# pangenome/seqrush

Hardware: AMD Instinct MI355X
Metric: aligned pairs/sec all-vs-all 64x5kb (higher is better)
Workload: dtype i16; 1 GPU; C2: 64 x 5 kb synthetic (5% SNP, seed 2001), all-vs-all incl. self = 4096 ordered pairs, -k 0 -S 0,5,8,2,24,1 --orientation-scores 0,1,1,1, biWFA (Ultralow); pairs_total=4096, pairs_per_gpu=4096, parallelism=pair-shard x1

## Files before the change

include/seqrush_amd.h:

```cpp
#ifndef SEQRUSH_AMD_H
#define SEQRUSH_AMD_H
#include <stddef.h>
#include <stdint.h>

#ifdef __cplusplus
extern "C" {
#endif

#define SR_ABI_VERSION 2

typedef enum {
    SR_OK = 0,
    SR_ERR_INVALID = -1,
    SR_ERR_NO_DEVICE = -2,
    SR_ERR_HIP = -3,
    SR_ERR_ALPHABET = -4,
    SR_ERR_EMPTY_SEQ = -5,
    SR_ERR_UNSUPPORTED = -6,
    SR_ERR_DEVICE_FAULT = -7,
    SR_ERR_IO = -8,
    SR_ERR_NOMEM = -9
} sr_status;

typedef struct {
// ... 116 lines not shown
    uint64_t random_entries;
    uint64_t random_processed;
    uint64_t random_aligned;
    uint64_t checks;
    uint64_t windows;
    uint64_t post_tree;
    uint64_t final_components;
    int32_t stabilized;
    int32_t tree_defaulted;
    uint32_t tree_k_nearest, tree_k_farthest;
    double tree_rand_frac;
    uint32_t tree_kmer;
    uint32_t reserved;
} sr_iter_stats;
int sr_ctx_load_iterative(sr_ctx *c, const sr_seqset *seqs, const sr_params *p, int keep_alignments);
int sr_ctx_run_iterative(sr_ctx *c);
int sr_ctx_iterative_stats(sr_ctx *c, sr_iter_stats *out, uint64_t *check_counts, uint64_t cap);
int sr_ctx_iterative_alignments(sr_ctx *c, sr_alignments **out);
int sr_uf_count_components_host(const uint64_t *nodes, uint64_t n, uint64_t total_len, uint64_t *count);
int sr_iterative_stop_host(const uint64_t *counts, uint64_t nchecks, uint64_t post_tree, uint64_t *stop_check);
int sr_iterative_pair_lists(uint32_t n, const uint8_t *sel, const sr_params *p, uint32_t **tree_i, uint32_t **tree_j,
                            uint64_t *tree_count, uint32_t **rand_i, uint32_t **rand_j, uint64_t *rand_count);
int sr_base_cone_reach(int e1, int e2, int two, int levels_left);
int sr_mirror_map(const uint32_t *query_idx, const uint32_t *target_idx, uint64_t count, const uint32_t *batch_first,
                  uint32_t nbatch, uint32_t workgroups, uint32_t *mirror_out, uint64_t *partners_out);
int sr_ctx_orientation_scores(sr_ctx *c, int32_t *fwd, int32_t *rev);
int sr_mirror_bt_pick(const int *off, int transposed);
int sr_mirror_bt_rank_transposed(int tag);
int sr_mirror_bt_tie_host(const int *off);
int sr_mirror_bp_pick_host(const int *val, const int *dist, const int *comp, const int *diag, int n, int value_bias,
                           int *pick_out, int *pick_t_out);
int sr_replay_record_ints(void);
void sr_replay_transpose_host(const int *rec, int *out);
int sr_replay_match_host(const int *recs, int nrec, const int *segs, int nseg, int level, int *match_out);

typedef struct {
    uint64_t min_size;
    int32_t keep_alignments;
    uint32_t join_below;
} sr_inv_params;
typedef struct {
    uint64_t scanned;
    uint64_t sites;
    uint64_t candidates;
    uint64_t accepted;
    uint64_t rejected_score;
// ... 217 lines not shown
```

seqrush_amd/_lib.py:

```python
import ctypes as C
import os

_HERE = os.path.dirname(os.path.abspath(__file__))
LIB_PATH = os.environ.get("SEQRUSH_AMD_LIB") or os.path.join(_HERE, "libseqrush_amd.so")

EXPORTS = [
    "sr_default_params", "sr_parse_scores", "sr_parse_orientation_scores",
    "sr_parse_sparsification", "sr_align_all", "sr_alignments_free", "sr_alignment_cigar",
    "sr_align_and_unite", "sr_uf_find", "sr_uf_same", "sr_write_paf", "sr_ctx_create",
    "sr_ctx_destroy", "sr_ctx_set_stream", "sr_ctx_load", "sr_ctx_reset_uf", "sr_ctx_align",
    "sr_ctx_unite", "sr_ctx_sync", "sr_ctx_alignments", "sr_ctx_download_uf", "sr_ctx_uf_size",
    "sr_ctx_num_pairs", "sr_ctx_dp_cells", "sr_ctx_labels_device", "sr_ctx_merge_labels",
    "sr_ctx_download_labels", "sr_ctx_kernel_ms", "sr_ctx_counters", "sr_build_gfa", "sr_free",
    "sr_last_error", "sr_abi_version", "sr_device_count", "sr_pair_list", "sr_ctx_align_kernel",
    "sr_ctx_load_paf", "sr_unite_paf", "sr_ctx_build_gfa", "sr_ctx_load_pairs", "sr_ctx_pairs",
    "sr_ctx_num_batches", "sr_ctx_workspace_report", "sr_ctx_run", "sr_ctx_align_all", "sr_ctx_pair_results",
    "sr_ctx_labels_device_u32", "sr_ctx_merge_labels_u32", "sr_ctx_counters_ext",
    "sr_build_gfa_opts", "sr_ctx_build_gfa_opts", "sr_ctx_merge_labels_host",
    "sr_uf_init_host", "sr_uf_unite_host", "sr_uf_merge_labels_host", "sr_uf_canonical_labels_host",
    "sr_build_gfa_from_nodes", "sr_ctx_counters_all", "sr_knobs_doc",
    "sr_sort_params_default", "sr_ctx_build_gfa_sorted", "sr_sort_gfa", "sr_sgd_layout", "sr_sgd_tables", "sr_sort_stats",
    "sr_ctx_load_iterative", "sr_ctx_run_iterative", "sr_ctx_iterative_stats", "sr_ctx_iterative_alignments",
    "sr_uf_count_components_host", "sr_iterative_stop_host", "sr_iterative_pair_lists", "sr_base_cone_reach",
    "sr_ctx_enable_inversions", "sr_ctx_inversion_stats", "sr_ctx_inversion_jobs", "sr_ctx_inversion_alignments",
    "sr_append_paf_tagged", "sr_inversion_sites_host", "sr_inversion_candidate", "sr_inversion_accept",
    "sr_inversion_scan_device",
    "sr_ctx_inversion_join_stats", "sr_inversion_sites_host_join", "sr_inversion_accept_site", "sr_inversion_scan_device_join",
    "sr_compact_gfa", "sr_compact_stats",
    "sr_sketch_device", "sr_knn_select_device",
    "sr_graph_stats_gfa", "sr_graph_stats_free", "sr_graph_stats_report", "sr_stats_sq_sums_host",
    "sr_mirror_map", "sr_mirror_bt_pick", "sr_mirror_bt_rank_transposed", "sr_mirror_bt_tie_host", "sr_mirror_bp_pick_host",
    "sr_ctx_orientation_scores",
    "sr_layout_params_default", "sr_layout_gfa", "sr_layout_tsv", "sr_layout_svg", "sr_layout_quality", "sr_layout_stats",
    "sr_layout_resolve", "sr_layout_select_host",
    "sr_path_bins_gfa", "sr_path_bins_free", "sr_path_bins_tsv", "sr_viz_params_default", "sr_path_bins_rgb", "sr_path_bins_png",
    "sr_growth_params_default", "sr_growth_gfa", "sr_growth_free", "sr_growth_groups", "sr_growth_expected", "sr_growth_fit",
    "sr_growth_report",
    "sr_variant_params_default", "sr_variants_gfa", "sr_variants_free", "sr_variants_vcf",
    "sr_ctx_tail_deferred", "sr_ctx_tail_timeline", "sr_tail_shape",
    "sr_replay_record_ints", "sr_replay_transpose_host", "sr_replay_match_host",
    "sr_ctx_prio_timeline", "sr_tile_prio_role_host", "sr_tile_prio_epoch_shift",
]


class SeqSetC(C.Structure):
    _fields_ = [("n", C.c_uint32), ("bases", C.c_char_p), ("offsets", C.POINTER(C.c_uint64)),
                ("names", C.POINTER(C.c_char_p))]


class ParamsC(C.Structure):
    _fields_ = [
        ("match_score", C.c_int32), ("mismatch_penalty", C.c_int32),
        ("gap_open1", C.c_int32), ("gap_ext1", C.c_int32),
        ("gap_open2", C.c_int32), ("gap_ext2", C.c_int32),
        ("ori_match", C.c_int32), ("ori_mismatch", C.c_int32),
        ("ori_gap_open", C.c_int32), ("ori_gap_ext", C.c_int32),
        ("min_match_len", C.c_uint64), ("max_divergence", C.c_double),
        ("exclude_self", C.c_int32), ("memory_mode", C.c_int32),
        ("sparsify_kind", C.c_int32), ("sparsify_factor", C.c_double),
        ("sparsify_seed", C.c_uint64), ("canonical_labels", C.c_int32), ("device", C.c_int32),
        ("shard_rank", C.c_uint32), ("shard_count", C.c_uint32),
        ("tree_k_nearest", C.c_uint32), ("tree_k_farthest", C.c_uint32), ("tree_rand_frac", C.c_double),
        ("tree_kmer", C.c_uint32),
    ]
# ... 186 lines not shown
    L.sr_build_gfa_opts.argtypes = [PS, C.POINTER(u64), i32, C.POINTER(vp), C.POINTER(u64), C.POINTER(u64)]
    L.sr_ctx_build_gfa_opts.argtypes = [vp, PS, i32, C.POINTER(vp), C.POINTER(u64), C.POINTER(u64)]
    L.sr_uf_init_host.argtypes = [C.POINTER(u64), u64, u64]
    L.sr_uf_unite_host.argtypes = [C.POINTER(u64), u64, u64, u64]
    L.sr_uf_merge_labels_host.argtypes = [C.POINTER(u64), u64, C.POINTER(u64), C.c_uint32]
    L.sr_uf_canonical_labels_host.argtypes = [C.POINTER(u64), u64, C.POINTER(u64)]
    L.sr_build_gfa_from_nodes.argtypes = [PS, C.POINTER(u64), i32, C.POINTER(vp), C.POINTER(u64), C.POINTER(u64)]
    SP, PD = C.POINTER(SortParamsC), C.POINTER(C.c_double)
    L.sr_sort_params_default.argtypes = [SP]; L.sr_sort_params_default.restype = None
    L.sr_ctx_build_gfa_sorted.argtypes = [vp, PS, i32, SP, C.POINTER(vp), C.POINTER(u64), C.POINTER(u64)]
    L.sr_sort_gfa.argtypes = [C.c_char_p, SP, C.POINTER(vp), C.POINTER(u64), C.POINTER(u64)]
    L.sr_sgd_layout.argtypes = [C.c_char_p, SP, PD, u64]
    L.sr_sgd_tables.argtypes = [C.c_char_p, SP, SP, C.POINTER(u64), PD, PD, PD, PD]
    L.sr_sort_stats.argtypes = [PD, C.c_uint32]
    L.sr_pair_list.argtypes = [C.c_uint32, PP, C.POINTER(C.POINTER(C.c_uint32)),
                               C.POINTER(C.POINTER(C.c_uint32)), C.POINTER(u64)]
    L.sr_ctx_load_iterative.argtypes = [vp, PS, PP, i32]
    L.sr_ctx_run_iterative.argtypes = [vp]
    L.sr_ctx_iterative_stats.argtypes = [vp, C.POINTER(IterStatsC), C.POINTER(u64), u64]
    L.sr_ctx_iterative_alignments.argtypes = [vp, C.POINTER(C.POINTER(AlignmentsC))]
    L.sr_uf_count_components_host.argtypes = [C.POINTER(u64), u64, u64, C.POINTER(u64)]
    L.sr_iterative_stop_host.argtypes = [C.POINTER(u64), u64, u64, C.POINTER(u64)]
    L.sr_base_cone_reach.argtypes = [C.c_int, C.c_int, C.c_int, C.c_int]
    PU32 = C.POINTER(C.POINTER(C.c_uint32))
    L.sr_iterative_pair_lists.argtypes = [C.c_uint32, C.POINTER(C.c_uint8), PP, PU32, PU32, C.POINTER(u64), PU32, PU32,
                                          C.POINTER(u64)]
    L.sr_ctx_enable_inversions.argtypes = [vp, C.POINTER(InvParamsC)]
    L.sr_ctx_inversion_stats.argtypes = [vp, C.POINTER(InvStatsC)]
    L.sr_ctx_inversion_jobs.argtypes = [vp, C.POINTER(C.POINTER(InvJobC)), C.POINTER(u64)]
    L.sr_ctx_inversion_alignments.argtypes = [vp, C.POINTER(C.POINTER(AlignmentsC))]
    L.sr_append_paf_tagged.argtypes = [C.POINTER(AlignmentsC), PS, C.c_char_p, C.c_char_p]
    L.sr_inversion_sites_host.argtypes = [C.POINTER(C.c_uint32), u64, u64, C.POINTER(C.POINTER(InvSiteC)), C.POINTER(u64)]
    L.sr_inversion_candidate.argtypes = [u64, u64, u64]
    L.sr_inversion_accept.argtypes = [C.c_int32, C.c_int32]
    L.sr_inversion_scan_device.argtypes = [i32, C.POINTER(C.c_uint32), C.POINTER(u64), u64, u64,
                                           C.POINTER(C.POINTER(InvSiteC)), C.POINTER(C.POINTER(u64)), C.POINTER(u64)]
    PI32 = C.POINTER(C.c_int32)
    L.sr_ctx_inversion_join_stats.argtypes = [vp, C.POINTER(u64)]
    L.sr_inversion_sites_host_join.argtypes = [C.POINTER(C.c_uint32), u64, u64, C.c_uint32, PP, C.POINTER(C.POINTER(InvSiteC)),
                                               C.POINTER(PI32), C.POINTER(u64)]
    L.sr_inversion_accept_site.argtypes = [C.c_int32, C.c_int32]
    L.sr_inversion_scan_device_join.argtypes = [i32, C.POINTER(C.c_uint32), C.POINTER(u64), u64, u64, C.c_uint32, PP, PI32, PI32,
                                                C.POINTER(C.POINTER(InvSiteC)), C.POINTER(C.POINTER(u64)), C.POINTER(PI32),
                                                C.POINTER(u64), C.POINTER(u64)]
    PU32P = C.POINTER(C.POINTER(C.c_uint32))
    L.sr_sketch_device.argtypes = [i32, PS, C.c_uint32, C.POINTER(C.POINTER(u64)), PU32P, PU32P, PU32P]
# ... 61 lines not shown
```

seqrush_amd/csrc/sr_align_blk.inc:

```
#include "sr_blk_rows.inc"
#include "sr_blk_tile.inc"
#include "sr_blk_pass.inc"
#include "sr_blk_phase2.inc"
#include "sr_blk_orient.inc"

#define K_SHIFT0 29
#define K_WIDTH0 64
struct KSeqs { int poff_f, poff_r, toff_f, toff_r, plen_all, tlen_all; };
__device__ __forceinline__ void kjob_set(int jid, int base, int pb, int pe, int tb, int te, int rev, int begin, int chk,
                                         int seg, const KSeqs &q) {
    bjob_set(jid, base, pb, pe, tb, te, 0, begin, chk, seg, rev ? q.poff_r : q.poff_f);
    BJob &b = b_sh.job[jid];
    b.shift = (pe - pb) + K_SHIFT0;
    b.pad0 = rev ? q.toff_r : q.toff_f;
    b.pad2 = 1;
    if (rev) { b.p0 = q.plen_all - pe; b.t0 = q.tlen_all - te; }
}
__device__ __forceinline__ int kjob_width(int plen, int tlen) { return (plen + tlen + K_WIDTH0) & ~3; }

#define SR_BLK_MIN_WAVES 4
template <typename OT, int NT, bool TWO, int B, int E1, int E2, bool PROF = false, int X = 0, int OE1 = 0, typename RT = OT>
__global__ void __launch_bounds__(NT, SR_BLK_MIN_WAVES) sr_align_blk_kernel(SrAlignArgs a) {
    const int tid = threadIdx.x;
    if (a.tail_mode == SR_TAIL_RUN && *a.tail_count == 0u) return;
// ... 259 lines not shown
                if (RFL(k_sh.rp_ntot) == 0) break;
                any_bp = true;
                if (tid == 0) k_sh.dg_nbp += (unsigned long long)k_sh.rp_ntot;
                if (nact == 0) {
                    if (tid == 0) k_sh.dg_steps += 2ull * (unsigned long long)k_sh.rp_ntot * B * (unsigned long long)k_sh.rp_maxp;
                    continue;
                }
                const unsigned long long tb0 = KTICK();
                const int njobs = 2 * nact;
                for (int s0i = 0; RFL(b_sh.nrunning) > 0; s0i += B) {
                    const int s0 = kopaque_s(s0i);
                    const unsigned long long q0 = KTICK();
                    blk_pass<OT, TWO, NT, B, E1, E2, PROF, X, OE1, RT, true>(RR, s0, pen, njobs, row_ld, row_st, s0 == 0);
                    const unsigned long long q1 = KTICK();
                    __syncthreads();
                    const unsigned long long q2 = KTICK();
                    tq_pass += q1 - q0; tq_bar += q2 - q1;
                    if (tid == 0) k_sh.dg_steps += (unsigned long long)njobs * B;
                    const int avail = s0 + B - 1;
                    const int tid_o = tid;
                    if (tid < 64) {
                        const int tid = (int)kopaque_v((unsigned)tid_o);
                        KPRIO_HI();
                        if (tid < njobs) {
#pragma unroll
                            for (int j = 0; j < B; j++) gmak[tid * BFS_MAK_SLOTS + (s0 + j) % depth] = k_sh.jak[j][tid];
                        }
                        const unsigned long long qc1 = KTICK();
                        int ph = 0, ph0 = 0;
                        if (tid < nact) {
                            BSeg &sg = b_sh.seg[tid];
                            ph = sg.phase; ph0 = ph;
                            const long long smax = 2LL * ((long long)pen.o1 * 2 + (long long)pen.e1 * (sg.max_ad + 1)) + 1024;
                            if (ph == 1) {
                                int score_f = sg.score_f, score_r = sg.score_r, last_fwd = sg.last_fwd, f_ak = sg.f_ak, r_ak = sg.r_ak;
                                const int max_ad = sg.max_ad;
                                for (int j = 0; j < B && ph == 1; j++) {
                                    const int s = s0 + j;
                                    const int akf = k_sh.jak[j][2 * tid], akr = k_sh.jak[j][2 * tid + 1];
                                    if (s == 0) {
                                        f_ak = akf; r_ak = akr;
                                        if (f_ak + r_ak >= max_ad) ph = 2;
                                    } else {
                                        score_f = s; f_ak = akf; last_fwd = 1;
                                        if (f_ak + r_ak >= max_ad) ph = 2;
                                        else {
                                            score_r = s; r_ak = akr; last_fwd = 0;
                                            if ((long long)score_f + score_r > smax) ph = 4;
                                            else if (f_ak + r_ak >= max_ad) ph = 2;
                                        }
                                    }
                                }
                                sg.score_f = score_f; sg.score_r = score_r; sg.last_fwd = last_fwd; sg.f_ak = f_ak; sg.r_ak = r_ak;
                                sg.phase = ph;
                            }
                        }
                        const unsigned long long qc2 = KTICK();
                        if (PROF && tid == 0) { k_sh.t_c1 += qc1 - q2; k_sh.t_c2 += qc2 - qc1; }
                        const unsigned long long m2 = __ballot(ph == 2);
                        const unsigned long long mnew = __ballot(ph == 2 && ph0 == 1);
                        if (tid == 0) k_sh.newmask = (unsigned)mnew;
                        if (tid == 0) { k_sh.p2mask_lo = (unsigned)m2; k_sh.p2mask_hi = (unsigned)(m2 >> 32); }
                        if (m2 == 0ull) {
                            const unsigned long long run = __ballot(ph == 1);
                            if (tid < nact && ph != 1) { b_sh.job[2 * tid].active = 0; b_sh.job[2 * tid + 1].active = 0; }
                            if (tid == 0) b_sh.nrunning = __popcll(run);
                            if (run != 0ull) blk_setup<TWO, NT, B, E1, E2, KTIGHT>(s0 + B, pen, njobs);
                        }
                        KPRIO_LO();
                    }
                    __syncthreads();
                    const unsigned long long q3 = KTICK();
                    tq_ctl += q3 - q2;
                    bool p2_or_rec = (RFL(k_sh.p2mask_lo) | RFL(k_sh.p2mask_hi)) != 0u;
                    if (a.lazy_id) {
                        if (RFL(k_sh.newmask) != 0u) p2_or_rec = true;
                        for (unsigned nm = RFL(k_sh.newmask); nm != 0u; nm &= nm - 1u) {
                            const int sa = __ffs((int)nm) - 1;
                            blk_recompute<OT, TWO, NT, B, E1, E2, X, OE1>(RR, pen, sa, RFL(b_sh.seg[sa].score_f), s0, row_ld, row_st);
                        }
                    }
                    tq_rec += KTICK() - q3;
                    if ((RFL(k_sh.p2mask_lo) | RFL(k_sh.p2mask_hi)) != 0u) {
                        blk_phase2<OT, TWO, NT, B, E1, E2, RT, PROF>(RR, clist, gmak, pen, s0, nact, gap_opening);
                        if (tid < 64) {
                            KPRIO_HI();
                            const int ph = (tid < nact) ? b_sh.seg[tid].phase : 0;
                            const unsigned long long run = __ballot(ph == 1 || ph == 2);
                            if (tid < nact && ph != 1 && ph != 2) { b_sh.job[2 * tid].active = 0; b_sh.job[2 * tid + 1].active = 0; }
                            if (tid == 0) b_sh.nrunning = __popcll(run);
                            if (run != 0ull) blk_setup<TWO, NT, B, E1, E2, KTIGHT>(s0 + B, pen, njobs);
                            KPRIO_LO();
                        }
                    }
                    const unsigned long long q4 = KTICK();
                    if (p2_or_rec) __syncthreads();
                    tq_ph2 += q4 - q3; tq_tail += KTICK() - q4;
                    if (tid == 0) k_sh.dg_npass += 1ull;
                }
                if (tid < nact) {
                    BSeg &sg = b_sh.seg[tid];
                    GP<int> e = cur + (size_t)sg.list_pos * SR_BFS_SEGREC;
                    const int sp = sg.pe - sg.pb, st = sg.te - sg.tb;
                    const int bh = sg.bp_off_f, bv = sg.bp_off_f - sg.bp_k_f;
                    if (sg.phase != 3 || sg.bp_score == INT_MAX) atomicOr(&b_sh.err, SR_DEV_ERR_SCORE_BOUND);
                    else if (bv < 0 || bv > sp || bh < 0 || bh > st) atomicOr(&b_sh.err, SR_DEV_ERR_BREAKPOINT);
                    else {
                        e[SL_BV] = bv; e[SL_BH] = bh; e[SL_BCOMP] = sg.bp_comp; e[SL_BSF] = sg.bp_score_f; e[SL_BSR] = sg.bp_score_r;
                        const int ri = k_sh.rp_nrec + tid;
                        if (k_sh.rp_record != 0 && ri < SR_BPREC_MAX) {
                            GP<int> r = (GP<int>)a.brec + (size_t)blockIdx.x * (SR_BPREC_MAX * SR_BPREC_INTS) + ri * SR_BPREC_INTS;
                            const unsigned long long cs = k_sh.cells_l[2 * tid] + k_sh.cells_l[2 * tid + 1] - (unsigned long long)(long long)k_sh.sg_sur[tid];
                            r[SR_BR_LEVEL] = k_sh.rp_level;
                            r[SR_BR_PB] = sg.pb; r[SR_BR_PE] = sg.pe; r[SR_BR_TB] = sg.tb; r[SR_BR_TE] = sg.te; r[SR_BR_CB] = sg.cb; r[SR_BR_CE] = sg.ce;
// ... 76 lines not shown
                        kjob_set(nb, 0, e[SL_PB], e[SL_PE], e[SL_TB], e[SL_TE], 0, e[SL_CB], ce, nb, ks);
                        b_sh.job[nb].shift = wj / 2;
                        b_sh.job[nb].pad1 = lj;
                        b_sh.job[nb].hbase = (unsigned)used; b_sh.job[nb].hw = (unsigned)wj;
                        b_sh.base_entry[nb] = p; b_sh.base_score[nb] = -1;
                        used += need; lmax = max(lmax, lj);
                        nb++;
                    }
                    b_sh.nbase = nb; b_sh.next_pos = p; b_sh.njobs = nb; b_sh.nrunning = nb;
                    b_sh.geom.hist_levels = lmax;
                }
                __syncthreads();
                int nb = RFL(b_sh.nbase);
                pos = RFL(b_sh.next_pos);
                if (nb > 0) {
                    if (tid == 0) k_sh.dg_nbase += (unsigned long long)nb;
                    const int hlevels = RFL(b_sh.geom.hist_levels);
                    for (int s0i = 0; RFL(b_sh.nrunning) > 0; s0i += B) {
                        const int s0 = kopaque_s(s0i);
                        if (s0 + B > hlevels) { if (tid == 0) b_sh.err |= SR_DEV_ERR_BASE_OVERFLOW; break; }
                        blk_pass<OT, TWO, NT, B, E1, E2, PROF, X, OE1, OT, false, true>(RH, s0, pen, nb, row_ld, row_st, s0 == 0);
                        __syncthreads();
                        if (tid == 0) k_sh.dg_steps += (unsigned long long)b_sh.nrunning * B;
                        if (tid < 64) {
                            KPRIO_HI();
                            bool running = false;
                            if (tid < nb && b_sh.job[tid].active) {
                                int hit = -1;
#pragma unroll
                                for (int l = B - 1; l >= 0; l--) if (k_sh.jreach[l][tid]) hit = l;
                                if (hit >= 0) {
                                    b_sh.base_score[tid] = s0 + hit; b_sh.job[tid].active = 0;
                                    atomicAdd(&b_sh.cells, (unsigned long long)(-blk_surplus(pen, tid, s0 + hit, s0 + B - 1)));
                                } else if (s0 + 2 * B > b_sh.job[tid].pad1) {
                                    GP<int> e = cur + (size_t)b_sh.base_entry[tid] * SR_BFS_SEGREC;
                                    b_sh.job[tid].active = 0;
                                    if (e[SL_REM] < 0 || b_sh.job[tid].pad1 >= a.hist_levels) atomicOr(&b_sh.err, SR_DEV_ERR_BASE_OVERFLOW);
                                    else { e[SL_REM] = -1; atomicMin(&k_sh.redo_from, tid); atomicAdd(&k_sh.dg_redo, 1ull); }
                                } else running = true;
                            }
                            const unsigned long long rm = __ballot(running);
                            if (tid == 0) b_sh.nrunning = __popcll(rm);
                            if (rm != 0ull) blk_setup<TWO, NT, B, E1, E2, false, true>(s0 + B, pen, nb);
                            KPRIO_LO();
                        }
                        __syncthreads();
                    }
                    __syncthreads();
                    const int redo = RFL(k_sh.redo_from);
                    if (redo < nb) {
                        if (tid == 0) k_sh.dg_nbase -= (unsigned long long)(nb - redo);
                        nb = redo; pos = RFL(b_sh.base_entry[redo]);
                    }
                    const unsigned long long tbt0 = KTICK();
                    if (tid < nb && RFL(b_sh.err) == 0) {
                        KPRIO_HI();
                        int n = 0;
                        const int e = bfs_backtrace<OT, TWO>(bhist + b_sh.job[tid].hbase, b_sh.job[tid].hw, tid, b_sh.base_score[tid],
                                                             btbuf + (size_t)tid * SR_BFS_BTCAP, &n);
                        b_sh.bt_n[tid] = n;
                        if (e & SR_MIRROR_BT_TIE) k_sh.mir_tie = 1;
                        if (e & ~SR_MIRROR_BT_TIE) atomicOr(&b_sh.err, e & ~SR_MIRROR_BT_TIE);
                        KPRIO_LO();
                    }
                    __syncthreads();
                    tb_bt += KTICK() - tbt0;
// ... 196 lines not shown
```

seqrush_amd/csrc/sr_blk_pass.inc:

```
#include "sr_base_cone.h"
#include "sr_prio_rule.h"
template <bool TWO, int E1, int E2>
__device__ __forceinline__ int kreach(const SrPen &p, int s, int begin) {
    int r;
    if (begin == SR_C_M) {
        r = (s >= p.o1 + E1) ? (s - p.o1) / E1 : 0;
        if (TWO && s >= p.o2 + E2) r = max(r, (s - p.o2) / E2);
    } else {
        r = s / E1;
        if (TWO) r = max(r, s / E2);
    }
    return r;
}

template <bool TWO, int B, int E1, int E2, bool TIGHT>
__device__ __forceinline__ void kwindow(const SrPen &pen, const BJob &b, int s0, int &glo, int &ghi) {
    const int Rw = kreach<TWO, E1, E2>(pen, s0 + B - 1, b.begin);
    const int mg = TIGHT ? 1 : pen.scope + 1;
    const int wlo = max(-b.plen - 1, -Rw - mg), whi = min(b.tlen + 1, Rw + mg);
    glo = (wlo + b.shift) >> 2; ghi = (whi + b.shift) >> 2;
}

#define KTICK() (PROF ? __builtin_amdgcn_s_memrealtime() : 0ull)
__device__ __forceinline__ void kprio_role() {
    switch (RFL(k_sh.prio_role)) {
    case 1: __builtin_amdgcn_s_setprio(1); break;
    case 2: __builtin_amdgcn_s_setprio(2); break;
    case 3: __builtin_amdgcn_s_setprio(3); break;
    default: __builtin_amdgcn_s_setprio(0); break;
    }
}
__device__ __forceinline__ void kprio_epoch() {
    const int wg = RFL(k_sh.prio_wg);
    if (wg > 1) {
        const unsigned epoch = (unsigned)(__builtin_amdgcn_s_memrealtime() >> SR_PRIO_EPOCH_SHIFT);
        if (threadIdx.x == 0) k_sh.prio_role = sr_tile_prio_role((unsigned)k_sh.prio_rank, epoch, (unsigned)wg);
    }
}
#define KPRIO_HI() __builtin_amdgcn_s_setprio(3)
#define KPRIO_LO() kprio_role()
#ifndef SR_BASE_CONE
#define SR_BASE_CONE 1
#endif
template <bool TWO, int NT, int B, int E1, int E2, bool TIGHT = false, bool BASE = false>
__device__ __forceinline__ void blk_setup(int s0, const SrPen &pen, int njobs) {
    const int tid = threadIdx.x;
    constexpr bool CONE = BASE && SR_BASE_CONE;
    int nt = 0, glo = 0, ghi = -1, cells = 0, ccells = 0;
    const bool act = tid < njobs && b_sh.job[tid].active;
    const int pglo = (tid < BJ_MAX) ? k_sh.jglo[tid] : 0, pghi = (tid < BJ_MAX) ? k_sh.jghi[tid] : -1;
    if (act) {
        const BJob &b = b_sh.job[tid];
        int Rw = 0, clo0 = 0, chi0 = 0;
#pragma unroll
        for (int j = 0; j < B; j++) {
            Rw = kreach<TWO, E1, E2>(pen, s0 + j, b.begin);
            int klo = max(-b.plen, -Rw), khi = min(b.tlen, Rw);
            cells += (khi >= klo) ? khi - klo + 1 : 0;
            if (CONE) {
                const int rb = sr_cone_reach(E1, E2, TWO, b.pad1 - 1 - (s0 + j));
                klo = max(klo, b.kend - rb); khi = min(khi, b.kend + rb);
                if (j == 0) { clo0 = b.kend - rb; chi0 = b.kend + rb; }
            }
            k_sh.jklo[j][tid] = klo; k_sh.jkhi[j][tid] = khi;
            ccells += (khi >= klo) ? khi - klo + 1 : 0;
        }
        (void)Rw;
        kwindow<TWO, B, E1, E2, TIGHT>(pen, b, s0, glo, ghi);
        if (CONE) {
            const int mg = TIGHT ? 1 : pen.scope + 1;
            const int wlo = max(max(-b.plen - 1, -Rw - mg), clo0 - 1), whi = min(min(b.tlen + 1, Rw + mg), chi0 + 1);
            glo = (wlo + b.shift) >> 2; ghi = (whi >= wlo) ? (whi + b.shift) >> 2 : glo - 1;
        }
        nt = max(0, (ghi - glo + KGeo<B>::OWN) / KGeo<B>::OWN);
        if (BASE && ccells) atomicAdd(&k_sh.base_cells, (unsigned long long)ccells);
    }
    int incl = nt, hincl = 0;
#pragma unroll
    for (int o = 1; o < 64; o <<= 1) {
        const int v = __shfl_up(incl, o, 64), h = __shfl_up(hincl, o, 64);
        if (tid >= o) { incl += v; hincl += h; }
    }
    if (tid < BJ_MAX) {
        k_sh.jglo[tid] = glo; k_sh.jghi[tid] = ghi;
        k_sh.jgplo[tid] = pglo; k_sh.jgphi[tid] = pghi;
        k_sh.jtstart[tid + 1] = incl;
        k_sh.jmerge[tid] = 0;
        k_sh.jband[tid] = INT_MAX / 2;
#pragma unroll
        for (int j = 0; j < B; j++) { k_sh.jak[j][tid] = 0; k_sh.jreach[j][tid] = 0; }
    }
    if (tid == 0) k_sh.jtstart[0] = 0;
    if (tid == 63) { k_sh.nband = hincl; k_sh.total_tiles = incl + hincl; k_sh.next_tile = NT / 64; if (BASE) k_sh.base_tiles += (unsigned long long)incl; }
    k_sh.cells_l[tid] += (unsigned long long)cells;
    kprio_epoch();
}

template <typename OT, bool TWO, int NT, int B, int E1, int E2, bool PROF, int X = 0, int OE1 = 0, typename ST = OT, bool RING = false, bool BASE = false>
__device__ __forceinline__ void blk_pass(const KRows<OT, ST> &R, int s0, const SrPen &pen, int njobs,
                                         unsigned &row_ld, unsigned &row_st, const bool setup = true) {
    const int tid = threadIdx.x;
    if (setup) {
        const unsigned long long tsu0 = KTICK();
        if (tid < 64) blk_setup<TWO, NT, B, E1, E2, RING && KTIGHT_OF(OT, ST, B, X), BASE>(s0, pen, njobs);
        __syncthreads();
        if (PROF && threadIdx.x == 0) k_sh.t_setup += KTICK() - tsu0;
    }
    kprio_role();
    const int total = RFL(k_sh.total_tiles);
    const int slot0 = kslots(R, s0);
    const int nband = RFL(k_sh.nband);
    for (int t = (tid >> 6); t < total;) {
        int lo, ti;
        if (t < nband) { lo = RFL(k_sh.jbandown[t]); ti = RFL(k_sh.jband[lo]); }
        else {
            const int r = t - nband;
            int hi = njobs; lo = 0;
            while (hi - lo > 1) { const int mid = (lo + hi) >> 1; if (RFL(k_sh.jtstart[mid]) <= r) lo = mid; else hi = mid; }
            ti = r - RFL(k_sh.jtstart[lo]);
            ti += (ti >= RFL(k_sh.jband[lo])) ? 1 : 0;
        }
        blk_tile_any<OT, TWO, B, E1, E2, false, X, OE1, ST, RING>(R, s0, slot0, pen, lo, ti, lo, row_ld, row_st);
        int nx = 0;
        if ((tid & 63) == 0) nx = atomicAdd(&k_sh.next_tile, 1);
        t = RFL(nx);
    }
}

template <typename OT, bool TWO, int NT, int B, int E1, int E2, int X = 0, int OE1 = 0, typename ST = OT>
__device__ __forceinline__ void blk_recompute(const KRows<OT, ST> &R, const SrPen &pen, int sa, int entry_level, int s0_now,
                                              unsigned &row_ld, unsigned &row_st) {
    const int tid = threadIdx.x;
    const int wlo = max(0, entry_level - pen.scope);
    for (int blk = (wlo / B) * B; blk <= s0_now; blk += B) {
        __syncthreads();
        if (tid < 2) {
            const BJob &b = b_sh.job[2 * sa + tid];
            int Rw = 0;
#pragma unroll
            for (int j = 0; j < B; j++) {
                Rw = kreach<TWO, E1, E2>(pen, blk + j, b.begin);
                k_sh.jklo[j][BJ_MAX + tid] = max(-b.plen, -Rw); k_sh.jkhi[j][BJ_MAX + tid] = min(b.tlen, Rw);
            }
            (void)Rw;
// ... 33 lines not shown
```

seqrush_amd/csrc/sr_blk_rows.inc:

```
#define SR_ORI_B 16
#define SR_KB_MAX 10
#define KB_LV (SR_ORI_B > SR_KB_MAX ? SR_ORI_B : SR_KB_MAX)
#define KB_MAX SR_KB_MAX
#define KPK_U16_OF(OT, ST, B, X) (sizeof(OT) == 4 && sizeof(ST) == 2 && (X) > 0 && (B) % 10 == 0)
#define KTIGHT_OF(OT, ST, B, X) ((X) > 0 && (B) % 10 == 0 && (sizeof(OT) == 2 || KPK_U16_OF(OT, ST, B, X)))

struct KShared {
    int jklo[KB_LV][BJ_MAX + 2], jkhi[KB_LV][BJ_MAX + 2];
    int jak[KB_MAX][BJ_MAX], jreach[KB_LV][BJ_MAX];
    int jtstart[BJ_MAX + 1], jglo[BJ_MAX + 2], jghi[BJ_MAX + 2];
    int jmerge[BJ_MAX];
    int jband[BJ_MAX], jbandown[BJ_MAX], nband;
    unsigned newmask;
    int rt_n0, rt_total;
    int jgplo[BJ_MAX + 2], jgphi[BJ_MAX + 2];
    int total_tiles;
    int next_tile;
    int prio_role, prio_rank, prio_wg;
    int p2n, p2seg[K_P2];
    unsigned p2mask_lo, p2mask_hi;
    int pc_n[K_P2], pc_s1[K_P2][2 * KB_MAX];
    unsigned char pc_side[K_P2][2 * KB_MAX];
    signed char pc_idx[K_P2][2][KB_MAX];
    unsigned long long pc_best[K_P2][2 * KB_MAX];
    unsigned long long pc_best_t[K_P2][2 * KB_MAX];
    int pu_start[2 * K_P2 + 1], pu_glo[2 * K_P2];
    int pu_kmin[2 * K_P2], pu_kmax[2 * K_P2];
    int cl_n;
#ifdef SR_BOUNDS
    unsigned lds_seq_bytes;
    int bnd_flag; unsigned bnd_off, bnd_ext, bnd_what;
#endif
    int mir_tie, mir_next;
    unsigned long long mir_snap[4];
    unsigned long long mir_pairs, mir_ties;
// ... 144 lines not shown
}

__device__ __forceinline__ int lane_left(int x) { return __builtin_amdgcn_update_dpp(NULLV, x, 0x138, 0xf, 0xf, false); }
__device__ __forceinline__ int lane_right(int x) { return __builtin_amdgcn_update_dpp(NULLV, x, 0x130, 0xf, 0xf, false); }
__device__ __forceinline__ int row16_max(int v) {
    v = max(v, __builtin_amdgcn_update_dpp(v, v, 0x111, 0xf, 0xf, false));
    v = max(v, __builtin_amdgcn_update_dpp(v, v, 0x112, 0xf, 0xf, false));
    v = max(v, __builtin_amdgcn_update_dpp(v, v, 0x114, 0xf, 0xf, false));
    v = max(v, __builtin_amdgcn_update_dpp(v, v, 0x118, 0xf, 0xf, false));
    return v;
}

__device__ __forceinline__ int row16_max_nn(int v) {
    v = max(v, __builtin_amdgcn_update_dpp(0, v, 0x111, 0xf, 0xf, true));
    v = max(v, __builtin_amdgcn_update_dpp(0, v, 0x112, 0xf, 0xf, true));
    v = max(v, __builtin_amdgcn_update_dpp(0, v, 0x114, 0xf, 0xf, true));
    v = max(v, __builtin_amdgcn_update_dpp(0, v, 0x118, 0xf, 0xf, true));
    return v;
}

template <int B> struct KGeo {
    static constexpr int HL = B <= 5 ? 2 : (B + 3) / 4;
    static constexpr int OWN = 64 - 2 * HL;
};
```

seqrush_amd/csrc/sr_host.cpp:

```cpp
#include <hip/hip_runtime_api.h>
#include <algorithm>
#include <chrono>
#include <climits>
#include <functional>
#include <queue>
#include <cmath>
#include <cstdio>
#include <cstdlib>
#include <cstring>
#include <string>
#include <unordered_map>
#include <unordered_set>
#include <vector>
#include "../../include/seqrush_amd.h"
#include "sr_internal.h"
#include "sr_graph.h"
#include "sr_sort.h"
#include "sr_compact.h"
#include "sr_iter_rule.h"
#include "sr_inv_rule.h"
#include "sr_base_cone.h"
#include "sr_mirror_rule.h"
#include "sr_prio_rule.h"

static thread_local std::string g_err;
static int fail(int code, const std::string &msg) { g_err = msg; return code; }
int sr_fail(int code, const std::string &msg) { return fail(code, msg); }
extern "C" const char *sr_last_error(void) { return g_err.c_str(); }

struct SrKnob { const char *name, *unset, *doc; };
static const SrKnob SR_KNOBS[] = {
    {"SR_ALIGN_IMPL", "2 when the penalties have a blocked instance", "1 = level-per-pass kernel (sr_align_bfs_kernel), 2 = score-blocked kernel"},
    {"SR_BLK_LEVELS", "10 for x=5, o1+e1=10", "5 = generic 5-level blocked instance instead of the exact 10-level one"},
    {"SR_ALIGN_THREADS", "by pairs per CU", "threads per workgroup: 64 | 128 | 256 | 512 | 1024"},
    {"SR_WG_PER_CU", "4", "workgroups per CU the launch is sized for"},
    {"SR_NWG", "CUs x workgroups per CU", "cap on workgroups (several pairs per workgroup on small inputs)"},
    {"SR_RING_U16", "1 below 57 k", "0 = 32-bit searches keep 32-bit ring rows"},
    {"SR_LAZY_ID", "1", "0 = searches store their I/D rows from the first level (no recompute pass)"},
    {"SR_HIST_JOBS", "4", "worst-case base cases the per-workgroup history holds (1..16)"},
    {"SR_BFS_BASE_JOBS", "16 (lean builds 4 / 8)", "base cases per batch"},
    {"SR_CIGAR_ARENA_OPS", "25 % of free memory", "CIGAR arena in ops (tests: force batches)"},
    {"SR_POISON_ROWS", "off", "fill the row workspaces with this offset before the run (stale-row tests)"},
    {"SR_PREORIENT", "by pairs per CU and LDS", "1 / 0 = orientation as its own kernel / inside the alignment kernel"},
    {"SR_NO_REORDER", "off", "keep list order instead of the cost-sorted dequeue order"},
    {"SR_ORIENT_LEVELS", "off", "orientation level by level even for the default penalties"},
    {"SR_NO_KBITS", "off", "no q-gram bound in the orientation kernel"},
// ... 2632 lines not shown
}
extern "C" int sr_uf_count_components_host(const uint64_t *nodes, uint64_t n, uint64_t total_len, uint64_t *count) {
    if (!nodes || !count || 2 * total_len > n) return fail(SR_ERR_INVALID, "bad node array");
    uint64_t c = 0;
    for (uint64_t x = 0; x < 2 * total_len; x++) c += (nodes[x] & UFH_MASK) == x;
    *count = c;
    return SR_OK;
}

extern "C" int sr_iterative_stop_host(const uint64_t *counts, uint64_t nchecks, uint64_t post_tree, uint64_t *stop_check) {
    if ((!counts && nchecks) || !stop_check) return fail(SR_ERR_INVALID, "null argument");
    SrIterState s{};
    s.prev = post_tree;
    *stop_check = 0;
    for (uint64_t k = 0; k < nchecks && !s.stopped; k++) sr_iter_step(&s, counts[k], (uint32_t)k);
    if (s.stopped) *stop_check = (uint64_t)s.stop_check + 1;
    return SR_OK;
}

extern "C" int sr_base_cone_reach(int e1, int e2, int two, int levels_left) {
    return sr_cone_reach(e1, e2, two != 0, levels_left);
}

extern "C" int sr_uf_canonical_labels_host(const uint64_t *nodes, uint64_t n, uint64_t *labels_out) {
    if (!nodes || !labels_out) return fail(SR_ERR_INVALID, "null argument");
    std::vector<uint64_t> root(n), mn(n, UINT64_MAX);
    for (uint64_t i = 0; i < n; i++) {
        const uint64_t r = sr_uf_find(nodes, n, i);
        if (r >= n) return fail(SR_ERR_INVALID, "node array is not a uf_rush forest");
        root[i] = r;
        if (mn[r] == UINT64_MAX) mn[r] = i;
    }
    for (uint64_t i = 0; i < n; i++) labels_out[i] = mn[root[i]];
    return SR_OK;
}

static int write_paf_impl(const sr_alignments *a, const sr_seqset *seqs, const char *path, const char *mode, const char *tag);
extern "C" int sr_write_paf(const sr_alignments *a, const sr_seqset *seqs, const char *path) {
    return write_paf_impl(a, seqs, path, "w", nullptr);
}
extern "C" int sr_append_paf_tagged(const sr_alignments *a, const sr_seqset *seqs, const char *path, const char *tag) {
    return write_paf_impl(a, seqs, path, "a", tag);
}
static int write_paf_impl(const sr_alignments *a, const sr_seqset *seqs, const char *path, const char *mode, const char *tag) {
    if (!a || !seqs || !path || !seqs->names) return fail(SR_ERR_INVALID, "null argument");
    FILE *f = fopen(path, mode);
// ... 181 lines not shown
```

Baseline: 101,500 pairs/s.

## Spread blk_setup level tables across lanes and drop band-split tile bookkeeping

The per-pass setup now fills the per-level k-range tables with one lane per (aligner, level) pair instead of one lane looping over all B levels. It replaces the 64-wide shfl_up scan with a DPP prefix scan sized to BJ_MAX, and removes the band-split tile map so tile lookup is a plain binary search. The phase-1 end-of-block check becomes branchless with vectorised shared loads. It also adds a host twin of the table rules for testing. Risks are extra atomics on cells_l and a different scan that relies on BJ_MAX being at most 32.

```diff
diff --git a/include/seqrush_amd.h b/include/seqrush_amd.h
--- a/include/seqrush_amd.h
+++ b/include/seqrush_amd.h
@@ -162,6 +162,9 @@
 int sr_iterative_pair_lists(uint32_t n, const uint8_t *sel, const sr_params *p, uint32_t **tree_i, uint32_t **tree_j,
                             uint64_t *tree_count, uint32_t **rand_i, uint32_t **rand_j, uint64_t *rand_count);
 int sr_base_cone_reach(int e1, int e2, int two, int levels_left);
+int sr_pass_tables_host(const int *pen6, int scope, int B, int tight, int base, int s0, int njobs, const int *jobs, int *klo,
+                        int *khi, long long *cells, long long *ccells, int *glo, int *ghi, int *nt, int *tstart);
+int sr_pass_tile_own(int B);
 int sr_mirror_map(const uint32_t *query_idx, const uint32_t *target_idx, uint64_t count, const uint32_t *batch_first,
                   uint32_t nbatch, uint32_t workgroups, uint32_t *mirror_out, uint64_t *partners_out);
 int sr_ctx_orientation_scores(sr_ctx *c, int32_t *fwd, int32_t *rev);
diff --git a/seqrush_amd/_lib.py b/seqrush_amd/_lib.py
--- a/seqrush_amd/_lib.py
+++ b/seqrush_amd/_lib.py
@@ -40,6 +40,7 @@
     "sr_ctx_tail_deferred", "sr_ctx_tail_timeline", "sr_tail_shape",
     "sr_replay_record_ints", "sr_replay_transpose_host", "sr_replay_match_host",
     "sr_ctx_prio_timeline", "sr_tile_prio_role_host", "sr_tile_prio_epoch_shift",
+    "sr_pass_tables_host", "sr_pass_tile_own",
 ]
 
 
@@ -272,6 +273,9 @@
     L.sr_uf_count_components_host.argtypes = [C.POINTER(u64), u64, u64, C.POINTER(u64)]
     L.sr_iterative_stop_host.argtypes = [C.POINTER(u64), u64, u64, C.POINTER(u64)]
     L.sr_base_cone_reach.argtypes = [C.c_int, C.c_int, C.c_int, C.c_int]
+    IP, LP = C.POINTER(C.c_int), C.POINTER(C.c_longlong)
+    L.sr_pass_tables_host.argtypes = [IP, C.c_int, C.c_int, C.c_int, C.c_int, C.c_int, C.c_int, IP, IP, IP, LP, LP, IP, IP, IP, IP]
+    L.sr_pass_tile_own.argtypes = [C.c_int]
     PU32 = C.POINTER(C.POINTER(C.c_uint32))
     L.sr_iterative_pair_lists.argtypes = [C.c_uint32, C.POINTER(C.c_uint8), PP, PU32, PU32, C.POINTER(u64), PU32, PU32,
                                           C.POINTER(u64)]
diff --git a/seqrush_amd/csrc/sr_align_blk.inc b/seqrush_amd/csrc/sr_align_blk.inc
--- a/seqrush_amd/csrc/sr_align_blk.inc
+++ b/seqrush_amd/csrc/sr_align_blk.inc
@@ -305,9 +305,15 @@
                     if (tid < 64) {
                         const int tid = (int)kopaque_v((unsigned)tid_o);
                         KPRIO_HI();
-                        if (tid < njobs) {
-#pragma unroll
-                            for (int j = 0; j < B; j++) gmak[tid * BFS_MAK_SLOTS + (s0 + j) % depth] = k_sh.jak[j][tid];
+                        {
+                            const int sb = s0 % depth, steps = sr_pass_steps(njobs, B);
+                            for (int st = 0; st < steps; st++) {
+                                int al, j;
+                                if (sr_pass_lane(tid, st, B, al, j) && al < njobs) {
+                                    const int sl = sb + j;
+                                    gmak[al * BFS_MAK_SLOTS + (sl >= depth ? sl - depth : sl)] = k_sh.jak[j][al];
+                                }
+                            }
                         }
                         const unsigned long long qc1 = KTICK();
                         int ph = 0, ph0 = 0;
@@ -318,20 +324,26 @@
                             if (ph == 1) {
                                 int score_f = sg.score_f, score_r = sg.score_r, last_fwd = sg.last_fwd, f_ak = sg.f_ak, r_ak = sg.r_ak;
                                 const int max_ad = sg.max_ad;
-                                for (int j = 0; j < B && ph == 1; j++) {
+                                typedef int __attribute__((ext_vector_type(2), may_alias)) I2;
+                                I2 ak[B];
+#pragma unroll
+                                for (int j = 0; j < B; j++) ak[j] = *(const I2 *)&k_sh.jak[j][2 * tid];
+#pragma unroll
+                                for (int j = 0; j < B; j++) {
                                     const int s = s0 + j;
-                                    const int akf = k_sh.jak[j][2 * tid], akr = k_sh.jak[j][2 * tid + 1];
+                                    const bool on = ph == 1;
+                                    const int akf = ak[j].x, akr = ak[j].y;
+                                    const bool both = akf + akr >= max_ad;
                                     if (s == 0) {
-                                        f_ak = akf; r_ak = akr;
-                                        if (f_ak + r_ak >= max_ad) ph = 2;
+                                        f_ak = on ? akf : f_ak; r_ak = on ? akr : r_ak;
+                                        ph = (on && both) ? 2 : ph;
                                     } else {
-                                        score_f = s; f_ak = akf; last_fwd = 1;
-                                        if (f_ak + r_ak >= max_ad) ph = 2;
-                                        else {
-                                            score_r = s; r_ak = akr; last_fwd = 0;
-                                            if ((long long)score_f + score_r > smax) ph = 4;
-                                            else if (f_ak + r_ak >= max_ad) ph = 2;
-                                        }
+                                        const bool fwd_hit = akf + r_ak >= max_ad;
+                                        const bool rev = on && !fwd_hit;
+                                        const bool over = (long long)s + s > smax;
+                                        score_f = on ? s : score_f; f_ak = on ? akf : f_ak; last_fwd = on ? (fwd_hit ? 1 : 0) : last_fwd;
+                                        score_r = rev ? s : score_r; r_ak = rev ? akr : r_ak;
+                                        ph = on ? (fwd_hit ? 2 : (over ? 4 : (both ? 2 : 1))) : ph;
                                     }
                                 }
                                 sg.score_f = score_f; sg.score_r = score_r; sg.last_fwd = last_fwd; sg.f_ak = f_ak; sg.r_ak = r_ak;
@@ -348,7 +360,7 @@
                             const unsigned long long run = __ballot(ph == 1);
                             if (tid < nact && ph != 1) { b_sh.job[2 * tid].active = 0; b_sh.job[2 * tid + 1].active = 0; }
                             if (tid == 0) b_sh.nrunning = __popcll(run);
-                            if (run != 0ull) blk_setup<TWO, NT, B, E1, E2, KTIGHT>(s0 + B, pen, njobs);
+                            if (run != 0ull) blk_setup<TWO, NT, B, E1, E2, KTIGHT>(s0 + B, pen, njobs, tid);
                         }
                         KPRIO_LO();
                     }
@@ -367,12 +379,13 @@
                     if ((RFL(k_sh.p2mask_lo) | RFL(k_sh.p2mask_hi)) != 0u) {
                         blk_phase2<OT, TWO, NT, B, E1, E2, RT, PROF>(RR, clist, gmak, pen, s0, nact, gap_opening);
                         if (tid < 64) {
+                            const int tid = (int)kopaque_v((unsigned)tid_o);
                             KPRIO_HI();
                             const int ph = (tid < nact) ? b_sh.seg[tid].phase : 0;
                             const unsigned long long run = __ballot(ph == 1 || ph == 2);
                             if (tid < nact && ph != 1 && ph != 2) { b_sh.job[2 * tid].active = 0; b_sh.job[2 * tid + 1].active = 0; }
                             if (tid == 0) b_sh.nrunning = __popcll(run);
-                            if (run != 0ull) blk_setup<TWO, NT, B, E1, E2, KTIGHT>(s0 + B, pen, njobs);
+                            if (run != 0ull) blk_setup<TWO, NT, B, E1, E2, KTIGHT>(s0 + B, pen, njobs, tid);
                             KPRIO_LO();
                         }
                     }
@@ -495,13 +508,17 @@
                         blk_pass<OT, TWO, NT, B, E1, E2, PROF, X, OE1, OT, false, true>(RH, s0, pen, nb, row_ld, row_st, s0 == 0);
                         __syncthreads();
                         if (tid == 0) k_sh.dg_steps += (unsigned long long)b_sh.nrunning * B;
+                        const int tid_o = tid;
                         if (tid < 64) {
+                            const int tid = (int)kopaque_v((unsigned)tid_o);
                             KPRIO_HI();
                             bool running = false;
                             if (tid < nb && b_sh.job[tid].active) {
-                                int hit = -1;
+                                int hit = -1, jr[B];
 #pragma unroll
-                                for (int l = B - 1; l >= 0; l--) if (k_sh.jreach[l][tid]) hit = l;
+                                for (int l = 0; l < B; l++) jr[l] = k_sh.jreach[l][tid];
+#pragma unroll
+                                for (int l = B - 1; l >= 0; l--) if (jr[l]) hit = l;
                                 if (hit >= 0) {
                                     b_sh.base_score[tid] = s0 + hit; b_sh.job[tid].active = 0;
                                     atomicAdd(&b_sh.cells, (unsigned long long)(-blk_surplus(pen, tid, s0 + hit, s0 + B - 1)));
@@ -514,7 +531,7 @@
                             }
                             const unsigned long long rm = __ballot(running);
                             if (tid == 0) b_sh.nrunning = __popcll(rm);
-                            if (rm != 0ull) blk_setup<TWO, NT, B, E1, E2, false, true>(s0 + B, pen, nb);
+                            if (rm != 0ull) blk_setup<TWO, NT, B, E1, E2, false, true>(s0 + B, pen, nb, tid);
                             KPRIO_LO();
                         }
                         __syncthreads();
diff --git a/seqrush_amd/csrc/sr_blk_pass.inc b/seqrush_amd/csrc/sr_blk_pass.inc
--- a/seqrush_amd/csrc/sr_blk_pass.inc
+++ b/seqrush_amd/csrc/sr_blk_pass.inc
@@ -1,24 +1,16 @@
 #include "sr_base_cone.h"
 #include "sr_prio_rule.h"
+#include "sr_pass_rule.h"
 template <bool TWO, int E1, int E2>
 __device__ __forceinline__ int kreach(const SrPen &p, int s, int begin) {
-    int r;
-    if (begin == SR_C_M) {
-        r = (s >= p.o1 + E1) ? (s - p.o1) / E1 : 0;
-        if (TWO && s >= p.o2 + E2) r = max(r, (s - p.o2) / E2);
-    } else {
-        r = s / E1;
-        if (TWO) r = max(r, s / E2);
-    }
-    return r;
+    return sr_pass_reach(p.o1, E1, p.o2, E2, TWO, s, begin == SR_C_M);
 }
 
 template <bool TWO, int B, int E1, int E2, bool TIGHT>
 __device__ __forceinline__ void kwindow(const SrPen &pen, const BJob &b, int s0, int &glo, int &ghi) {
-    const int Rw = kreach<TWO, E1, E2>(pen, s0 + B - 1, b.begin);
-    const int mg = TIGHT ? 1 : pen.scope + 1;
-    const int wlo = max(-b.plen - 1, -Rw - mg), whi = min(b.tlen + 1, Rw + mg);
-    glo = (wlo + b.shift) >> 2; ghi = (whi + b.shift) >> 2;
+    int nt;
+    sr_pass_window(kreach<TWO, E1, E2>(pen, s0 + B - 1, b.begin), TIGHT ? 1 : pen.scope + 1, b.plen, b.tlen, b.shift, false, 0, 0,
+                   KGeo<B>::OWN, glo, ghi, nt);
 }
 
 #define KTICK() (PROF ? __builtin_amdgcn_s_memrealtime() : 0ull)
@@ -42,57 +34,67 @@
 #ifndef SR_BASE_CONE
 #define SR_BASE_CONE 1
 #endif
+__device__ __forceinline__ int kscan_jobs(int v) {
+    static_assert(BJ_MAX <= 32 && BJ_MAX % 4 == 0, "kscan_jobs: at most two DPP rows of aligners");
+    v += __builtin_amdgcn_update_dpp(0, v, 0x111, 0xf, 0xf, true);
+    v += __builtin_amdgcn_update_dpp(0, v, 0x112, 0xf, 0xf, true);
+    v += __builtin_amdgcn_update_dpp(0, v, 0x114, 0xf, 0xf, true);
+    if (BJ_MAX > 8) v += __builtin_amdgcn_update_dpp(0, v, 0x118, 0xf, 0xf, true);
+    if (BJ_MAX > 16) v += __builtin_amdgcn_update_dpp(0, v, 0x142, 0xa, 0xf, false);
+    return v;
+}
 template <bool TWO, int NT, int B, int E1, int E2, bool TIGHT = false, bool BASE = false>
-__device__ __forceinline__ void blk_setup(int s0, const SrPen &pen, int njobs) {
-    const int tid = threadIdx.x;
+__device__ __forceinline__ void blk_setup(int s0, const SrPen &pen, int njobs, const int tid) {
     constexpr bool CONE = BASE && SR_BASE_CONE;
-    int nt = 0, glo = 0, ghi = -1, cells = 0, ccells = 0;
+    if (tid < BJ_MAX) {
+#pragma unroll
+        for (int j = 0; j < B; j++) { k_sh.jak[j][tid] = 0; k_sh.jreach[j][tid] = 0; }
+    }
+    if (BASE) {
+        if (tid < njobs && b_sh.job[tid].active) {
+            const BJob &b = b_sh.job[tid];
+            int cells = 0, ccells = 0;
+#pragma unroll
+            for (int j = 0; j < B; j++) {
+                const int rb = CONE ? sr_cone_reach(E1, E2, TWO, b.pad1 - 1 - (s0 + j)) : 0;
+                int klo, khi, c, cc;
+                sr_pass_level(kreach<TWO, E1, E2>(pen, s0 + j, b.begin), b.plen, b.tlen, CONE, CONE ? b.kend : 0, rb, klo, khi, c, cc);
+                k_sh.jklo[j][tid] = klo; k_sh.jkhi[j][tid] = khi;
+                cells += c; ccells += cc;
+            }
+            k_sh.cells_l[tid] += (unsigned long long)cells;
+            if (ccells) atomicAdd(&k_sh.base_cells, (unsigned long long)ccells);
+        }
+    } else {
+        const int steps = sr_pass_steps(njobs, B);
+        for (int st = 0; st < steps; st++) {
+            int a, j;
+            if (sr_pass_lane(tid, st, B, a, j) && a < njobs && b_sh.job[a].active) {
+                const BJob &b = b_sh.job[a];
+                int klo, khi, cells, ccells;
+                sr_pass_level(kreach<TWO, E1, E2>(pen, s0 + j, b.begin), b.plen, b.tlen, false, 0, 0, klo, khi, cells, ccells);
+                k_sh.jklo[j][a] = klo; k_sh.jkhi[j][a] = khi;
+                if (cells) atomicAdd(&k_sh.cells_l[a], (unsigned long long)cells);
+            }
+        }
+    }
+    int nt = 0, glo = 0, ghi = -1;
     const bool act = tid < njobs && b_sh.job[tid].active;
     const int pglo = (tid < BJ_MAX) ? k_sh.jglo[tid] : 0, pghi = (tid < BJ_MAX) ? k_sh.jghi[tid] : -1;
     if (act) {
         const BJob &b = b_sh.job[tid];
-        int Rw = 0, clo0 = 0, chi0 = 0;
-#pragma unroll
-        for (int j = 0; j < B; j++) {
-            Rw = kreach<TWO, E1, E2>(pen, s0 + j, b.begin);
-            int klo = max(-b.plen, -Rw), khi = min(b.tlen, Rw);
-            cells += (khi >= klo) ? khi - klo + 1 : 0;
-            if (CONE) {
-                const int rb = sr_cone_reach(E1, E2, TWO, b.pad1 - 1 - (s0 + j));
-                klo = max(klo, b.kend - rb); khi = min(khi, b.kend + rb);
-                if (j == 0) { clo0 = b.kend - rb; chi0 = b.kend + rb; }
-            }
-            k_sh.jklo[j][tid] = klo; k_sh.jkhi[j][tid] = khi;
-            ccells += (khi >= klo) ? khi - klo + 1 : 0;
-        }
-        (void)Rw;
-        kwindow<TWO, B, E1, E2, TIGHT>(pen, b, s0, glo, ghi);
-        if (CONE) {
-            const int mg = TIGHT ? 1 : pen.scope + 1;
-            const int wlo = max(max(-b.plen - 1, -Rw - mg), clo0 - 1), whi = min(min(b.tlen + 1, Rw + mg), chi0 + 1);
-            glo = (wlo + b.shift) >> 2; ghi = (whi >= wlo) ? (whi + b.shift) >> 2 : glo - 1;
-        }
-        nt = max(0, (ghi - glo + KGeo<B>::OWN) / KGeo<B>::OWN);
-        if (BASE && ccells) atomicAdd(&k_sh.base_cells, (unsigned long long)ccells);
+        const int rb0 = CONE ? sr_cone_reach(E1, E2, TWO, b.pad1 - 1 - s0) : 0;
+        sr_pass_window(kreach<TWO, E1, E2>(pen, s0 + B - 1, b.begin), TIGHT ? 1 : pen.scope + 1, b.plen, b.tlen, b.shift, CONE,
+                       CONE ? b.kend : 0, rb0, KGeo<B>::OWN, glo, ghi, nt);
     }
-    int incl = nt, hincl = 0;
-#pragma unroll
-    for (int o = 1; o < 64; o <<= 1) {
-        const int v = __shfl_up(incl, o, 64), h = __shfl_up(hincl, o, 64);
-        if (tid >= o) { incl += v; hincl += h; }
-    }
+    const int incl = kscan_jobs(nt);
     if (tid < BJ_MAX) {
         k_sh.jglo[tid] = glo; k_sh.jghi[tid] = ghi;
         k_sh.jgplo[tid] = pglo; k_sh.jgphi[tid] = pghi;
         k_sh.jtstart[tid + 1] = incl;
-        k_sh.jmerge[tid] = 0;
-        k_sh.jband[tid] = INT_MAX / 2;
-#pragma unroll
-        for (int j = 0; j < B; j++) { k_sh.jak[j][tid] = 0; k_sh.jreach[j][tid] = 0; }
     }
-    if (tid == 0) k_sh.jtstart[0] = 0;
-    if (tid == 63) { k_sh.nband = hincl; k_sh.total_tiles = incl + hincl; k_sh.next_tile = NT / 64; if (BASE) k_sh.base_tiles += (unsigned long long)incl; }
-    k_sh.cells_l[tid] += (unsigned long long)cells;
+    if (tid == 0) { k_sh.jtstart[0] = 0; k_sh.next_tile = (int)kopaque_v((unsigned)(NT / 64)); }
+    if (tid == BJ_MAX - 1) { k_sh.total_tiles = incl; if (BASE) k_sh.base_tiles += (unsigned long long)incl; }
     kprio_epoch();
 }
 
@@ -102,24 +104,17 @@
     const int tid = threadIdx.x;
     if (setup) {
         const unsigned long long tsu0 = KTICK();
-        if (tid < 64) blk_setup<TWO, NT, B, E1, E2, RING && KTIGHT_OF(OT, ST, B, X), BASE>(s0, pen, njobs);
+        if (tid < 64) blk_setup<TWO, NT, B, E1, E2, RING && KTIGHT_OF(OT, ST, B, X), BASE>(s0, pen, njobs, (int)kopaque_v((unsigned)tid));
         __syncthreads();
         if (PROF && threadIdx.x == 0) k_sh.t_setup += KTICK() - tsu0;
     }
     kprio_role();
     const int total = RFL(k_sh.total_tiles);
     const int slot0 = kslots(R, s0);
-    const int nband = RFL(k_sh.nband);
     for (int t = (tid >> 6); t < total;) {
-        int lo, ti;
-        if (t < nband) { lo = RFL(k_sh.jbandown[t]); ti = RFL(k_sh.jband[lo]); }
-        else {
-            const int r = t - nband;
-            int hi = njobs; lo = 0;
-            while (hi - lo > 1) { const int mid = (lo + hi) >> 1; if (RFL(k_sh.jtstart[mid]) <= r) lo = mid; else hi = mid; }
-            ti = r - RFL(k_sh.jtstart[lo]);
-            ti += (ti >= RFL(k_sh.jband[lo])) ? 1 : 0;
-        }
+        int hi = njobs, lo = 0;
+        while (hi - lo > 1) { const int mid = (lo + hi) >> 1; if (RFL(k_sh.jtstart[mid]) <= t) lo = mid; else hi = mid; }
+        const int ti = t - RFL(k_sh.jtstart[lo]);
         blk_tile_any<OT, TWO, B, E1, E2, false, X, OE1, ST, RING>(R, s0, slot0, pen, lo, ti, lo, row_ld, row_st);
         int nx = 0;
         if ((tid & 63) == 0) nx = atomicAdd(&k_sh.next_tile, 1);
diff --git a/seqrush_amd/csrc/sr_blk_rows.inc b/seqrush_amd/csrc/sr_blk_rows.inc
--- a/seqrush_amd/csrc/sr_blk_rows.inc
+++ b/seqrush_amd/csrc/sr_blk_rows.inc
@@ -1,3 +1,4 @@
+#include "sr_pass_rule.h"
 #define SR_ORI_B 16
 #define SR_KB_MAX 10
 #define KB_LV (SR_ORI_B > SR_KB_MAX ? SR_ORI_B : SR_KB_MAX)
@@ -7,10 +8,9 @@
 
 struct KShared {
     int jklo[KB_LV][BJ_MAX + 2], jkhi[KB_LV][BJ_MAX + 2];
-    int jak[KB_MAX][BJ_MAX], jreach[KB_LV][BJ_MAX];
+    alignas(8) int jak[KB_MAX][BJ_MAX];
+    int jreach[KB_LV][BJ_MAX];
     int jtstart[BJ_MAX + 1], jglo[BJ_MAX + 2], jghi[BJ_MAX + 2];
-    int jmerge[BJ_MAX];
-    int jband[BJ_MAX], jbandown[BJ_MAX], nband;
     unsigned newmask;
     int rt_n0, rt_total;
     int jgplo[BJ_MAX + 2], jgphi[BJ_MAX + 2];
@@ -201,4 +201,5 @@
 template <int B> struct KGeo {
     static constexpr int HL = B <= 5 ? 2 : (B + 3) / 4;
     static constexpr int OWN = 64 - 2 * HL;
+    static_assert(OWN == sr_pass_own(B), "sr_pass_rule.h: the host twin of the pass tables counts tiles with the same geometry");
 };
diff --git a/seqrush_amd/csrc/sr_host.cpp b/seqrush_amd/csrc/sr_host.cpp
--- a/seqrush_amd/csrc/sr_host.cpp
+++ b/seqrush_amd/csrc/sr_host.cpp
@@ -22,6 +22,7 @@
 #include "sr_base_cone.h"
 #include "sr_mirror_rule.h"
 #include "sr_prio_rule.h"
+#include "sr_pass_rule.h"
 
 static thread_local std::string g_err;
 static int fail(int code, const std::string &msg) { g_err = msg; return code; }
@@ -2700,6 +2701,40 @@
     return sr_cone_reach(e1, e2, two != 0, levels_left);
 }
 
+#define SR_PASS_JOB_INTS 7
+extern "C" int sr_pass_tile_own(int B) { return sr_pass_own(B); }
+extern "C" int sr_pass_tables_host(const int *pen6, int scope, int B, int tight, int base, int s0, int njobs, const int *jobs,
+                                   int *klo, int *khi, long long *cells, long long *ccells, int *glo, int *ghi, int *nt, int *tstart) {
+    if (!pen6 || !jobs || B < 1 || B > SR_PASS_LANES || njobs < 0 || pen6[2] < 1 || (pen6[5] && pen6[4] < 1)) return -1;
+    const int o1 = pen6[1], e1 = pen6[2], o2 = pen6[3], e2 = pen6[4];
+    const bool two = pen6[5] != 0, cone = base != 0;
+    const int steps = sr_pass_steps(njobs, B);
+    for (int st = 0; st < steps; st++)
+        for (int lane = 0; lane < SR_PASS_LANES; lane++) {
+            int a, j;
+            if (!sr_pass_lane(lane, st, B, a, j) || a >= njobs) continue;
+            const int *b = jobs + (size_t)a * SR_PASS_JOB_INTS;
+            if (!b[0]) continue;
+            const int rb = cone ? sr_cone_reach(e1, e2, two, b[6] - 1 - (s0 + j)) : 0;
+            int lo, hi, c, cc;
+            sr_pass_level(sr_pass_reach(o1, e1, o2, e2, two, s0 + j, b[1] == SR_C_M), b[2], b[3], cone, cone ? b[5] : 0, rb, lo, hi, c, cc);
+            klo[(size_t)j * njobs + a] = lo; khi[(size_t)j * njobs + a] = hi;
+            cells[a] += c; ccells[a] += cc;
+        }
+    tstart[0] = 0;
+    for (int a = 0; a < njobs; a++) {
+        const int *b = jobs + (size_t)a * SR_PASS_JOB_INTS;
+        glo[a] = 0; ghi[a] = -1; nt[a] = 0;
+        if (b[0]) {
+            const int rb0 = cone ? sr_cone_reach(e1, e2, two, b[6] - 1 - s0) : 0;
+            sr_pass_window(sr_pass_reach(o1, e1, o2, e2, two, s0 + B - 1, b[1] == SR_C_M), tight ? 1 : scope + 1, b[2], b[3], b[4], cone,
+                           cone ? b[5] : 0, rb0, sr_pass_own(B), glo[a], ghi[a], nt[a]);
+        }
+        tstart[a + 1] = tstart[a] + nt[a];
+    }
+    return steps;
+}
+
 extern "C" int sr_uf_canonical_labels_host(const uint64_t *nodes, uint64_t n, uint64_t *labels_out) {
     if (!nodes || !labels_out) return fail(SR_ERR_INVALID, "null argument");
     std::vector<uint64_t> root(n), mn(n, UINT64_MAX);
diff --git a/seqrush_amd/csrc/sr_pass_rule.h b/seqrush_amd/csrc/sr_pass_rule.h
--- /dev/null
+++ b/seqrush_amd/csrc/sr_pass_rule.h
@@ -0,0 +1,50 @@
+#pragma once
+
+#if defined(__HIPCC__) || defined(__CUDACC__)
+#define SR_PASS_HD __host__ __device__ __forceinline__
+#else
+#define SR_PASS_HD inline
+#endif
+
+#define SR_PASS_LANES 64
+
+SR_PASS_HD constexpr int sr_pass_own(int B) { return 64 - 2 * (B <= 5 ? 2 : (B + 3) / 4); }
+
+SR_PASS_HD int sr_pass_reach(int o1, int e1, int o2, int e2, bool two, int s, bool from_m) {
+    int r;
+    if (from_m) {
+        r = (s >= o1 + e1) ? (s - o1) / e1 : 0;
+        if (two && s >= o2 + e2) { const int r2 = (s - o2) / e2; r = r2 > r ? r2 : r; }
+    } else {
+        r = s / e1;
+        if (two) { const int r2 = s / e2; r = r2 > r ? r2 : r; }
+    }
+    return r;
+}
+
+SR_PASS_HD bool sr_pass_lane(int lane, int step, int B, int &aligner, int &level) {
+    const int per = SR_PASS_LANES / B, al = lane / B;
+    aligner = step * per + al; level = lane - al * B;
+    return al < per;
+}
+SR_PASS_HD int sr_pass_steps(int njobs, int B) { const int per = SR_PASS_LANES / B; return (njobs + per - 1) / per; }
+
+SR_PASS_HD void sr_pass_level(int Rw, int plen, int tlen, bool cone, int kend, int rb, int &klo, int &khi, int &cells, int &ccells) {
+    klo = -plen > -Rw ? -plen : -Rw; khi = tlen < Rw ? tlen : Rw;
+    cells = (khi >= klo) ? khi - klo + 1 : 0;
+    if (cone) {
+        klo = klo > kend - rb ? klo : kend - rb; khi = khi < kend + rb ? khi : kend + rb;
+    }
+    ccells = (khi >= klo) ? khi - klo + 1 : 0;
+}
+
+SR_PASS_HD void sr_pass_window(int Rw, int mg, int plen, int tlen, int shift, bool cone, int kend, int rb0, int own,
+                               int &glo, int &ghi, int &nt) {
+    int wlo = -plen - 1 > -Rw - mg ? -plen - 1 : -Rw - mg, whi = tlen + 1 < Rw + mg ? tlen + 1 : Rw + mg;
+    if (cone) {
+        wlo = wlo > kend - rb0 - 1 ? wlo : kend - rb0 - 1; whi = whi < kend + rb0 + 1 ? whi : kend + rb0 + 1;
+        glo = (wlo + shift) >> 2; ghi = (whi >= wlo) ? (whi + shift) >> 2 : glo - 1;
+    } else { glo = (wlo + shift) >> 2; ghi = (whi + shift) >> 2; }
+    nt = (ghi - glo + own) / own;
+    nt = nt > 0 ? nt : 0;
+}
```

Result: faster. 106,000 pairs/s (median of 6 runs) (+4.5%).
